# heracles-ec/heracles

Hardware: AMD Instinct MI355X
Metric: map->Cl pairs/sec + mixing-matrix build sec, nside=4096 lmax=6144 (higher is better)
Workload: dtype f64

## Files before the change

### heracles_amd/_lib.py

```python

from __future__ import annotations

import ctypes as C
import os
import threading

import numpy as np

_HERE = os.path.dirname(os.path.abspath(__file__))
_LIBNAME = os.environ.get("HX_LIBRARY") or os.path.join(_HERE, "libhxsht.so")
_lock = threading.Lock()
_lib = None

HX_OK = 0
HX_ERR_ARG, HX_ERR_NO_DEVICE, HX_ERR_HIP, HX_ERR_MEM, HX_ERR_UNSUPPORTED = -1, -2, -3, -4, -5

SYMBOLS = (
    "hx_version", "hx_last_error", "hx_device_count", "hx_init", "hx_set_stream",
    "hx_get_stream", "hx_set_async", "hx_synchronize", "hx_timer_start", "hx_timer_stop",
    "hx_profile_enable", "hx_profile_reset", "hx_profile_get", "hx_plan_create", "hx_set_max_lds_fft",
    "hx_plan_destroy", "hx_plan_scratch_bytes", "hx_plan_release_scratch", "hx_plan_set_leadin_resume", "hx_plan_set_leadin_cap", "hx_set_scratch_budget", "hx_plan_last_chunks", "hx_plan_mfma_flops", "hx_plan_executed_flops", "hx_executed_flops", "hx_measure_peaks", "hx_measured_mfma_clock", "hx_map2alm", "hx_map2alm_multi", "hx_map2alm_list", "hx_alm2map", "hx_copy",
    "hx_alm2cl_pairs", "hx_alm2cl_pairs_range", "hx_gauss_legendre", "hx_gauss_legendre_dd", "hx_wigner_d_table", "hx_mixmat",
    "hx_mixmat_eb", "hx_mixmat_eb_spin", "hx_mixmat_batch", "hx_mixctx_create", "hx_mixctx_apply", "hx_mixctx_apply_spin", "hx_mixctx_destroy", "hx_mixctx_set_bins", "hx_mixctx_apply_binned", "hx_mixctx_apply_binned_spin", "hx_cl2corr", "hx_corr2cl", "hx_cl2corr_cols", "hx_corr2cl_cols", "hx_cl2corr_cols_spin", "hx_corr2cl_cols_spin", "hx_xi_ratio", "hx_ang2pix_ring", "hx_map_values", "hx_ud_grade", "hx_reorder", "hx_matvec", "hx_pinv", "hx_alm_resample", "hx_region_maps", "hx_alm_subtract", "hx_fits_unpack_f64", "hx_fits_pack_f64", "hx_fits_unpack_columns",
    "hx_pointsht_create", "hx_pointsht_destroy", "hx_pointsht_info", "hx_pointsht_adjoint",
    "hx_pointsht_synthesis", "hx_pointsht_grids", "hx_pointgrid_gather", "hx_pointgrid_destroy",
    "hx_pixel_weights_size", "hx_pixel_weights_expand", "hx_pixel_weights_solve",
    "hx_ring_modes_size", "hx_ring_modes", "hx_legendre_from_modes", "hx_allgather_alms", "hx_host_alloc", "hx_host_free", "hx_mixmat_gemm_clock", "hx_mixmat_release", "hx_release_caches",
    "hx_cov_gram", "hx_cov_delete2", "hx_cov_shrink_sums",
    "hx_catmap_create", "hx_catmap_page", "hx_catmap_moments", "hx_catmap_finish", "hx_catmap_destroy",
    "hx_catalm_create", "hx_catalm_page", "hx_catalm_moments", "hx_catalm_finish", "hx_catalm_destroy",
    "hx_catmap_create_sel", "hx_catmap_page_sel", "hx_catmap_moments_sel", "hx_catmap_finish_sel", "hx_catmap_destroy_sel",
)


class HxError(RuntimeError):

# ... 24 lines not shown
        L = C.CDLL(_LIBNAME)
        vp, i, dp = C.c_void_p, C.c_int, C.c_void_p
        L.hx_version.restype = C.c_char_p
        L.hx_last_error.restype = C.c_char_p
        L.hx_get_stream.restype = vp
        L.hx_set_stream.argtypes = [vp]
        L.hx_plan_create.restype = vp
        L.hx_plan_create.argtypes = [i, i, i]
        L.hx_plan_destroy.argtypes = [vp]
        L.hx_plan_destroy.restype = None
        L.hx_plan_scratch_bytes.argtypes = [vp]
        L.hx_plan_scratch_bytes.restype = C.c_int64
        L.hx_plan_release_scratch.argtypes = [vp]
        L.hx_plan_set_leadin_resume.argtypes = [vp, i]
        L.hx_plan_set_leadin_cap.argtypes = [vp, C.c_int64]
        L.hx_set_scratch_budget.argtypes = [C.c_double]
        L.hx_plan_last_chunks.argtypes = [vp]
        L.hx_plan_mfma_flops.argtypes = [vp, i, i, C.POINTER(C.c_double)]
        L.hx_plan_executed_flops.argtypes = [vp, i, i, C.POINTER(C.c_double)]
        L.hx_executed_flops.argtypes = [C.POINTER(C.c_double), i]
        L.hx_measure_peaks.argtypes = [C.POINTER(C.c_double)]
        L.hx_measured_mfma_clock.restype = C.c_double
        L.hx_map2alm.argtypes = [vp, i, i, dp, dp, dp, dp, dp, i]
        L.hx_alm2map.argtypes = [vp, i, i, dp, dp]
        L.hx_map2alm_multi.argtypes = [vp, i, vp, vp, vp, vp, dp, dp, vp]
        L.hx_map2alm_list.argtypes = [vp, i, vp, vp, vp, dp, dp, dp, dp, i]
        L.hx_copy.argtypes = [vp, vp, C.c_int64]
        L.hx_alm2cl_pairs.argtypes = [i, vp, vp, i, i, vp, vp, dp]
        L.hx_alm2cl_pairs_range.argtypes = [i, vp, vp, i, i, vp, vp, i, i, i, dp]
        L.hx_gauss_legendre.argtypes = [i, dp, dp]
# ... 244 lines not shown
```

### heracles_amd/csrc/hx_analysis.hip

```cpp
#include <algorithm>
#include <cmath>
#include <cstdlib>
#include <cstring>

#include "hx_sht_common.h"

namespace hx {
using namespace hxfft;

constexpr int HALF_F = 1;
template <int SPIN>
struct LegCfg {
    static constexpr int NW = SPIN == 0 ? 16 : 8;
    static constexpr int NT = SPIN == 0 ? 1 : 2;
    static constexpr int NOP = SPIN == 0 ? 1 : 2;
    static constexpr int NPAR = (SPIN == 2 && HALF_F) ? 1 : 2;
};
int analysis_f_rows(int spin) { return spin == 0 ? LegCfg<0>::NPAR * LegCfg<0>::NOP : LegCfg<2>::NPAR * LegCfg<2>::NOP; }

struct LegParams {
    PlanDev P;
    const LegTask *__restrict__ tasks;
    const double *__restrict__ F;
    double *__restrict__ partial;
    int m0, ms;
    long long row0;
    int ng;
    int ncol;
    int pcol;
    const MTasks *__restrict__ of_m;
    const long long *__restrict__ arow;
    long long arow0;
    int add_all;
    const double *__restrict__ leadin;
    LegTask *tasks_out;
    double *leadin_out;
};

constexpr int COMB_NXCD = 8, COMB_XG = 4;
constexpr int COMB_TM = 16;
constexpr int COMB_IPT = 3;
constexpr int COMB_MPAD = 2;
static int combine_rp(int rowlen) { return rowlen <= 40 ? 8 : 4; }
static size_t combine_lds_bytes(int rp, int rowlen)
{
    return (size_t)COMB_TM * ((size_t)rp * rowlen + COMB_MPAD) * sizeof(double) + (size_t)COMB_TM * rp * sizeof(RingAtM) + COMB_TM * sizeof(int);
}
template <int SPIN, int RP>
__global__ __launch_bounds__(1024) void k_fourier_combine(PlanDev P, const double2 *__restrict__ Y, int ncomp, int ncol, int m0, int ms,
                                                         int nm, int kshift, int gx, int gy, const double *__restrict__ rw,
                                                         const LegTask *__restrict__ tasks, const MTasks *__restrict__ of_m,
// ... 121 lines not shown
template <int SPIN>
struct PipeCfg {
    static constexpr int NW = 4;
    static constexpr int RBS = SPIN == 0 ? 2 : 1;
    static constexpr int NCH = SPIN == 0 ? 2 : 1;
    static constexpr int NOP = SPIN == 0 ? 1 : 2;
};

__device__ __host__ inline int pipe_rho(int q, int k) { return 4 * q + k; }
__device__ __host__ inline int pipe_tile_idx(int c, int r) { return c * 32 + ((r ^ (c & 7)) * 2); }

constexpr int DUO_GAP = -1;
constexpr int DUO_PRIO = 1;
constexpr int DUO_ORDER = -1;
constexpr int DUO_SCALE_BITS2 = 100;
constexpr int DUO_SCALE_BITS0 = 300;

template <int K>
__device__ __forceinline__ double row_bcast(double v)
{
    double d;
    asm("v_mov_b64_dpp %0, %1 row_newbcast:%2 row_mask:0xf bank_mask:0xf" : "=v"(d) : "v"(v), "n"(K));
    return d;
}

template <int K>
__device__ __forceinline__ double row_bcast_fmac(double t, double p, double x)
{
    asm("v_fmac_f64_dpp %0, %1, %2 row_newbcast:%3 row_mask:0xf bank_mask:0xf" : "+v"(t) : "v"(p), "v"(x), "n"(K));
    return t;
}
// ... 84 lines not shown
    auto lds_barrier = []() __attribute__((always_inline)) {
        __builtin_amdgcn_s_waitcnt(0xc07f);
        __builtin_amdgcn_s_barrier();
    };
    int n_mf = 0, n_rec = 0;
    if (DUO_PRIO) __builtin_amdgcn_s_setprio(3);
    const int ti0 = SCOUT ? (int)blockIdx.y : 0, tis = SCOUT ? (int)gridDim.y : 1;
    for (int ti = ti0; ti < mt.count; ti += tis) {
        const LegTask task = SCOUT ? A.tasks_out[mt.first + ti] : A.tasks[mt.first + ti];
        first_group = ti == 0 && !A.add_all;
        const int bres = (RESUME && !SCOUT && A.leadin) ? task.pad : 0;
        int tid = threadIdx.x;
        asm volatile("; ring group" : "+v"(tid));
        const int w = tid >> 6, lane = tid & 63;
        const int ai = lane & 15, ak = lane >> 4;
        if (ti != ti0) __syncthreads();
        if (!SCOUT && bres > 0) {
            if (first_group) {
                double2 *z = reinterpret_cast<double2 *>(A.partial + orow * A.pcol);
                const long long nz = (long long)bres * LBLK * A.pcol / 2;
                for (long long i = tid; i < nz; i += 256) z[i] = make_double2(0.0, 0.0);
                asm volatile("s_waitcnt vmcnt(0)" ::: "memory");
            }
            if (bres >= nblk) continue;
        }

        const int rbi = SPIN == 0 ? 2 * w + (lane >> 5) : w;
        const int rpl = (task.rb0 + rbi) * RBLK + (lane & 31);
        const bool valid = rbi < task.nrb && rpl < P.nrp;
        const double x = valid ? P.z[rpl] : 0.0;
// ... 116 lines not shown
            return __all(dead) ? 1 : (__all(live) ? 3 : 2);
        };
        using I1 = std::integral_constant<int, 1>;
        using I2 = std::integral_constant<int, 2>;
        using I3 = std::integral_constant<int, 3>;

        const int fcol = tid & 15, fch = (tid >> 4) & 7, fpos = (tid >> 7) & 1;
        const int frow = (fch >> 1) + 8 * (fch & 1);
        const int qrow = tid / (4 * NXA), qcol = tid % (4 * NXA);
        double *pgrp = A.partial + (orow + (long long)bres * LBLK + 2 * frow + fpos) * A.pcol + fcol;
        double *pquad = A.partial + (orow + (long long)bres * LBLK + 2 * qrow) * A.pcol + NG * NCOL + qcol;
        double2 cnext[2] = {cfm[bres * LBLK], cfm[bres * LBLK + 16]};
        bool started = first_group;
        int nflush = 0;
        int woke = nblk;
        double svc[NCH], svp[NCH];
        int ssc[NCH];
        for (int b0 = bres; b0 < nblk; b0 += NSUB) {
            double4_t acc[NSUB][NG][2];
            double accx[NSUB][NXA][2];
            bool mine = false;
            if (SCOUT) {
#pragma unroll
                for (int c = 0; c < NCH; ++c) { svc[c] = vc[c]; svp[c] = vp[c]; ssc[c] = sc[c]; }
            }
#pragma unroll
            for (int sub = 0; sub < NSUB; ++sub) {
                const int b = b0 + sub;
#pragma unroll
                for (int g = 0; g < NG; ++g) acc[sub][g][0] = acc[sub][g][1] = (double4_t){0.0, 0.0, 0.0, 0.0};
#pragma unroll
                for (int g = 0; g < NXA; ++g) accx[sub][g][0] = accx[sub][g][1] = 0.0;
                if (b >= nblk) break;
                int rm = set_mode(b);
                const double2 cl[2] = {cnext[0], cnext[1]};
                if (rm == 3) recursion(I3{}, cl);
                else if (rm == 2) {
                    recursion(I2{}, cl);
                    if (SB != 300) {
                        bool lv = valid && sc[0] == 0;
                        if (NCH == 2) lv = lv || (valid && sc[NCH - 1] == 0);
                        if (!__any(lv)) rm = 1;
                    }
                } else recursion(I1{}, cl);
                cnext[0] = cfm[(b + 1) * LBLK];
                cnext[1] = cfm[(b + 1) * LBLK + 16];
                n_rec = __builtin_amdgcn_readfirstlane(n_rec + 1);
                mine = mine || rm >= 2;
                if (!SCOUT && rm >= 2) {
                    n_mf = __builtin_amdgcn_readfirstlane(n_mf + 1);
                    if (DUO_PRIO) __builtin_amdgcn_s_setprio(0);
                    constexpr int PF = 3;
                    auto a_fetch = [&](int sp) __attribute__((always_inline)) {
                        const int op = SPIN == 0 ? 0 : sp & 1, q = SPIN == 0 ? sp : sp >> 1;
                        const int c = SPIN == 0 ? (q >> 3) * 32 + pipe_rho(q & 7, ak) : op * 32 + pipe_rho(q, ak);
                        return *reinterpret_cast<const double2 *>(tw + pipe_tile_idx(c, ai));
                    };
                    double2 aq[PF + 1];
#pragma unroll
// ... 39 lines not shown
                                }
                            } else {
#pragma unroll
                                for (int g = 0; g < NG; ++g) acc[sub][g][pos] = __builtin_amdgcn_mfma_f64_16x16x4f64(a, fr[sp][HALFB ? 0 : pos][g], acc[sub][g][pos], 0, 0, 0);
#pragma unroll
                                for (int g = 0; g < NBX; ++g) accx[sub][g][pos] = __builtin_amdgcn_mfma_f64_4x4x4f64(a, frx[sp][HALFB ? 0 : pos][g], accx[sub][g][pos], 0, 0, 0);
                            }
                        }
                        __builtin_amdgcn_sched_barrier(0);
                    }
                    if (DUO_PRIO) __builtin_amdgcn_s_setprio(3);
                }
            }
            const bool two = NSUB > 1 && b0 + 1 < nblk;
            if (SCOUT) {
                if (lane == 0) lead_in[nflush & 1][w] = mine ? 1 : 0;
                lds_barrier();
                const int4 fl = *reinterpret_cast<const int4 *>(&lead_in[nflush & 1][0]);
                ++nflush;
                if (__builtin_amdgcn_readfirstlane(fl.x | fl.y | fl.z | fl.w) != 0) {
                    woke = b0;
                    break;
                }
                continue;
            }
            if (!started) {
                if (lane == 0) lead_in[nflush & 1][w] = mine ? 1 : 0;
                lds_barrier();
                const int4 fl = *reinterpret_cast<const int4 *>(&lead_in[nflush & 1][0]);
                ++nflush;
                started = __builtin_amdgcn_readfirstlane(fl.x | fl.y | fl.z | fl.w) != 0;
                if (!started) {
                    pgrp += (long long)NSUB * LBLK * A.pcol;
                    pquad += (long long)NSUB * LBLK * A.pcol;
                    continue;
                }
            }
#pragma unroll
// ... 25 lines not shown
                    put(pgrp + rsub + g * NCOL + 8 * (long long)A.pcol, (s4[0].y + s4[1].y) + (s4[2].y + s4[3].y));
                }
                if (NBX > 0 && tid < 64 * NBX) {
                    double2 s4[NW];
#pragma unroll
                    for (int ww = 0; ww < NW; ++ww) s4[ww] = *reinterpret_cast<const double2 *>(&tile[0][0] + ww * TW + sub * DSZ + DQ0 + tid * 2);
                    put(pquad + rsub, (s4[0].x + s4[1].x) + (s4[2].x + s4[3].x));
                    put(pquad + rsub + A.pcol, (s4[0].y + s4[1].y) + (s4[2].y + s4[3].y));
                }
            }
            pgrp += (long long)NSUB * LBLK * A.pcol;
            pquad += (long long)NSUB * LBLK * A.pcol;
            lds_barrier();
        }
        if (SCOUT) {
            if (woke > 0 && woke < nblk) {
                double *st = A.leadin_out + (long long)(mt.first + ti) * (NCH * 640) + tid;
#pragma unroll
                for (int c = 0; c < NCH; ++c) {
                    st[c * 640] = svc[c];
                    st[c * 640 + 256] = svp[c];
                    reinterpret_cast<int *>(st + c * 640 + 512 - tid)[tid] = ssc[c];
                }
            }
            if (tid == 0) A.tasks_out[mt.first + ti].pad = woke;
        }
    }
    if (!SCOUT && (threadIdx.x & 63) == 0) {
        atomicAdd(&g_exec_flops[0], (unsigned long long)n_mf * (32ull * (NG * 2048ull + NBX * 512ull)));
        atomicAdd(&g_exec_flops[1], (unsigned long long)n_rec * (64ull * LBLK * 4ull));
    }
// ... 135 lines not shown
        else return fail(HX_ERR_ARG, "legendre analysis: no two-group kernel for %d groups + %d blocks", sh.ng, sh.nbx);
        return HX_OK;
    }
    if (key == 10) hipLaunchKernelGGL((k_legendre_duo<SPIN, 1, 0, 2>), pgrid, db, 0, st, A, cn);
    else if (key == 11) hipLaunchKernelGGL((k_legendre_duo<SPIN, 1, 1, 2>), pgrid, db, 0, st, A, cn);
    else if (key == 20 && SPIN == 2) hipLaunchKernelGGL((k_legendre_duo<2, 2, 0, 2>), pgrid, db, 0, st, A, cn);
    else if (key == 12 && SPIN == 2) hipLaunchKernelGGL((k_legendre_duo<2, 1, 2, 2>), pgrid, db, 0, st, A, cn);
    else if (key == 21 && SPIN == 2) hipLaunchKernelGGL((k_legendre_duo<2, 2, 1, 2>), pgrid, db, 0, st, A, cn);
    else if (key == 20) hipLaunchKernelGGL((k_legendre_duo<SPIN, 2, 0>), pgrid, db, 0, st, A, cn);
    else if (key == 22 && SPIN == 2) hipLaunchKernelGGL((k_legendre_duo<2, 2, 2>), pgrid, db, 0, st, A, cn);
    else return fail(HX_ERR_ARG, "legendre analysis: no two-group kernel for %d groups + %d blocks", sh.ng, sh.nbx);
    return HX_OK;
}

constexpr long long LEADIN_CAP_BYTES = 8LL << 30;
static int leadin_table(hx_plan *pl, int spin, hx_plan::SpinData &sd, hx_plan::TaskSet &ts, const double **tab)
{
    *tab = nullptr;
    if (pl->leadin_resume < (spin == 0 ? 2 : 1) || ts.tasks.empty() || ts.leadin_skip) return HX_OK;
    if (ts.d_leadin.p) {
        *tab = ts.d_leadin.as<double>();
        return HX_OK;
    }
    const size_t per_task = (size_t)(spin == 0 ? PipeCfg<0>::NCH : PipeCfg<2>::NCH) * 640 * sizeof(double);
    const size_t bytes = ts.tasks.size() * per_task;
    size_t cap = (size_t)(pl->leadin_cap > 0 ? pl->leadin_cap : LEADIN_CAP_BYTES), fr = 0, tot = 0;
    if (hipMemGetInfo(&fr, &tot) == hipSuccess) cap = std::min(cap, fr / 10);
    else (void)hipGetLastError();
    if (bytes > cap) {
        ts.leadin_skip = true;
        return HX_OK;
    }
    if (ts.d_leadin.alloc(bytes) != HX_OK) {
        (void)hipGetLastError();
        ts.leadin_skip = true;
        return HX_OK;
    }
    LegParams A;
    A.P = pl->dev(); A.tasks = nullptr; A.F = nullptr; A.partial = nullptr;
    A.m0 = 0; A.ms = 1; A.row0 = 0; A.ng = 1; A.ncol = NCOL; A.pcol = NCOL;
    A.of_m = ts.d_of_m.as<MTasks>(); A.arow = ts.d_arow.as<long long>(); A.arow0 = 0; A.add_all = 1;
    A.leadin = nullptr; A.tasks_out = ts.d_tasks.as<LegTask>(); A.leadin_out = ts.d_leadin.as<double>();
    const dim3 grid((unsigned)(pl->lmax + 1), 8), db(256);
    if (spin == 0) hipLaunchKernelGGL((k_legendre_duo<0, 1, 0, 2, true>), grid, db, 0, rt().stream, A, sd.cn.as<double2>());
    else hipLaunchKernelGGL((k_legendre_duo<2, 1, 0, 2, true>), grid, db, 0, rt().stream, A, sd.cn.as<double2>());
    if (hipGetLastError() != hipSuccess) {
        ts.d_leadin.release();
        return fail(HX_ERR_HIP, "leadin_table: the scout launch failed");
    }
    *tab = ts.d_leadin.as<double>();
    return HX_OK;
}

static void launch_alm_reduce(hx_plan *pl, int spin, hx_plan::TaskSet &ts, long long row0, int m0, int ms, int nm, int nb, int ng, int pcol,
                              const double *d_fl, int add, double2 *d_alms, const double *al)
{
    const PlanDev P = pl->dev();
    const long long *arow = al ? ts.d_arow.as<long long>() : nullptr;
    if (spin == 0)
        hipLaunchKernelGGL(k_alm_reduce<0>, dim3(nm), dim3(256), 0, rt().stream, P, ts.d_tasks.as<LegTask>(), ts.d_of_m.as<MTasks>(), pl->partial.as<double>(),
                           row0, m0, ms, nb, ng, pcol, d_fl, add, d_alms, pl->nlm, arow, al);
    else
        hipLaunchKernelGGL(k_alm_reduce<2>, dim3(nm), dim3(256), 0, rt().stream, P, ts.d_tasks.as<LegTask>(), ts.d_of_m.as<MTasks>(), pl->partial.as<double>(),
                           row0, m0, ms, nb, ng, pcol, d_fl, add, d_alms, pl->nlm, arow, al);
}

template <int SPIN>
static int launch_chunk(hx_plan *pl, hx_plan::SpinData &sd, hx_plan::TaskSet &ts, int m0, int m1, int nb, const SweepShape &sh, const double *d_rw,
                        const double *d_fl, int add, double2 *d_alms, const double *leadin)
{
    const int ng = sh.ng + (sh.nbx > 0 ? 1 : 0), ncol = sh.ncol;
    const int pcol = sweep_pcol(sh);
    hipStream_t st = rt().stream;
    PlanDev P = pl->dev();
    const int t0 = ts.of_m[m0].first;
    const int t1 = ts.of_m[m1 - 1].first + ts.of_m[m1 - 1].count;
    const int ms = std::max(pl->m_step, 1), nm = (m1 - m0 + ms - 1) / ms;
    {
        ProfScope ps("fourier_combine");
        launch_fourier_combine<SPIN>(st, P, pl->Y.as<double2>(), nb, ncol, m0, ms, nm, d_rw, ts.d_tasks.as<LegTask>(), ts.d_of_m.as<MTasks>(),
                                     pl->F.as<double>(), 0, pl->nrp_pad / 32);
    }
    if (t1 > t0) {
        ProfScope ps("legendre_analysis");
        ProfScope ps2(SPIN == 0 ? "legendre_analysis_s0" : "legendre_analysis_s2");
        LegParams A;
        A.P = P; A.tasks = ts.d_tasks.as<LegTask>() + t0; A.F = pl->F.as<double>(); A.partial = pl->partial.as<double>();
        A.m0 = m0; A.ms = ms; A.row0 = ts.rows_before_m[m0]; A.ng = ng; A.ncol = ncol; A.pcol = pcol;
        A.of_m = ts.d_of_m.as<MTasks>(); A.arow = ts.d_arow.as<long long>(); A.arow0 = ts.arow[m0]; A.add_all = 0;
        A.tasks = ts.d_tasks.as<LegTask>();
        A.leadin = leadin; A.tasks_out = nullptr; A.leadin_out = nullptr;
        HX_TRY(launch_duo<SPIN>(sh, dim3((unsigned)nm), st, A, sd.cn.as<double2>()));
    }
    {
        ProfScope ps("alm_reduce");
        launch_alm_reduce(pl, SPIN, ts, ts.arow[m0], m0, ms, nm, nb, ng, pcol, d_fl, add, d_alms, sd.al.as<double>());
    }
    HX_HIP(hipGetLastError());
    return HX_OK;
}

static bool valu_batch(int spin, int nb) { return sweep_shape(spin, nb).valu != 0; }

static double analysis_budget(const hx_plan *pl)
{
    if (scratch_budget_bytes() > 0.0) return scratch_budget_bytes();
// ... 71 lines not shown
        return analysis_batch_valu(pl, spin, nb, d_maps, d_alms, d_rw, d_pw, d_fl, add, true);
    }
    if (valu_batch(spin, nb)) return analysis_batch_valu(pl, spin, nb, d_maps, d_alms, d_rw, d_pw, d_fl, add);
    const SweepShape sh = sweep_shape(spin, nb);
    hx_plan::TaskSet *ts = nullptr;
    hx_plan::SpinData *sd = nullptr;
    HX_TRY(spin_data(pl, spin, false, &sd));
    HX_TRY(task_set(pl, spin, false, one_set_task_blocks(spin), &ts));
    if (pl->hsrc == nullptr && pl->nssrc == nullptr) {
        HX_TRY(pl->Y.alloc(sizeof(double2) * (size_t)pl->ny * nb));
        HX_TRY(launch_ring_subdft_maps(pl, nb, d_maps, d_pw, pl->Y.as<double2>()));
    }
    std::vector<std::pair<int, int>> chunks;
    HX_TRY(plan_m_chunks(pl, (double)pl->nrp_pad * analysis_f_rows(spin) * sh.ncol * sizeof(double), ts->arow, sweep_pcol(sh) * sizeof(double), chunks));
    const double *leadin = nullptr;
    HX_TRY(leadin_table(pl, spin, *sd, *ts, &leadin));
    for (auto &ch : chunks) {
        if (spin == 0)
            HX_TRY(launch_chunk<0>(pl, *sd, *ts, ch.first, ch.second, nb, sh, d_rw, d_fl, add, d_alms, leadin));
        else
            HX_TRY(launch_chunk<2>(pl, *sd, *ts, ch.first, ch.second, nb, sh, d_rw, d_fl, add, d_alms, leadin));
    }
    return HX_OK;
}

bool analysis_can_stream(hx_plan *pl, int spin, int nb)
{
    if (!pl || pl->nside < 1 || pl->hsrc || pl->nssrc || pl->m_lo != 0 || pl->m_hi >= 0 || pl->m_step > 1) return false;
    if (nb < 1 || nb > analysis_max_comp(spin)) return false;
    const SweepShape sh = sweep_shape(spin, nb);
    if (!duo_shape(sh) || sh.valu) return false;
    const double f_bytes = (double)pl->nrp_pad * analysis_f_rows(spin) * sh.ncol * sizeof(double) * (pl->lmax + 1.0);
    const double p_bytes = 0.5 * (pl->lmax + 1.0) * (pl->lmax + 2.0 + LBLK) * sweep_pcol(sh) * sizeof(double);
    double budget = 80e9;
    if (scratch_budget_bytes() > 0.0) budget = scratch_budget_bytes();
    if (f_bytes + p_bytes > budget) return false;
// ... 4 lines not shown
    }
    const double y_bytes = (double)pl->ny * nb * sizeof(double2), stage_bytes = 2.0 * nb * (double)pl->npix * sizeof(double);
    const double held = (double)pl->F.bytes + (double)pl->partial.bytes + (double)pl->Y.bytes + (double)pl->stage[0].bytes + (double)pl->stage[1].bytes +
                        (double)pl->stage[2].bytes;
    return f_bytes + p_bytes + y_bytes + stage_bytes <= 0.95 * ((double)fr + held);
}

int analysis_stream_plan(hx_plan *pl, int spin, int nb, int nslab, StreamSweep &s)
{
    if (!analysis_can_stream(pl, spin, nb)) return fail(HX_ERR_ARG, "analysis_stream_plan: not a streamable sweep");
    HX_TRY(spin_data(pl, spin, false, &s.sd));
    HX_TRY(task_set(pl, spin, false, one_set_task_blocks(spin), &s.ts));
    hx_plan::TaskSet &ts = *s.ts;
    const SweepShape sh = sweep_shape(spin, nb);
    s.leadin = nullptr;
    s.pl = pl; s.spin = spin; s.nb = nb;
    const int nrb = (pl->nrp + RBLK - 1) / RBLK;
    std::vector<double> cum(nrb + 1, 0.0);
    for (int rb = 0; rb < nrb; ++rb) {
        double px = 0.0;
        for (int rp = rb * RBLK; rp < std::min((rb + 1) * RBLK, pl->nrp); ++rp) px += (rp == pl->nrp - 1 ? 4.0 : 8.0) * pl->h_nsub[rp];
        cum[rb + 1] = cum[rb] + px;
    }
    nslab = std::max(1, std::min(nslab, nrb));
    s.rp_edge.assign(1, 0);
    for (int k = 1; k < nslab; ++k) {
        const int rb = (int)(std::lower_bound(cum.begin(), cum.end(), cum[nrb] * k / nslab) - cum.begin());
        if (rb * RBLK > s.rp_edge.back() && rb < nrb) s.rp_edge.push_back(rb * RBLK);
    }
    s.rp_edge.push_back(nrb * RBLK);
// ... 7 lines not shown
            const int rb_hi = s.rp_edge[k + 1] / RBLK;
            MTasks &o = tab[(size_t)k * (lmax + 1) + m];
            o.first = t;
            while (t < mt.first + mt.count && ts.tasks[t].rb0 + ts.tasks[t].nrb <= rb_hi) ++t;
            o.count = t - o.first;
        }
        if (t != mt.first + mt.count) return fail(HX_ERR_ARG, "analysis_stream_plan: ring groups of m = %d left over", m);
    }
    HX_TRY(upload(s.d_of_m, tab));
    HX_TRY(pl->Y.alloc(sizeof(double2) * (size_t)pl->ny * nb));
    HX_TRY(pl->F.alloc((size_t)pl->nrp_pad * analysis_f_rows(spin) * sh.ncol * sizeof(double) * (size_t)(lmax + 1)));
    HX_TRY(pl->partial.alloc((size_t)ts.arow[lmax + 1] * sweep_pcol(sh) * sizeof(double)));
    return HX_OK;
}

int analysis_stream_leadin(StreamSweep &s) { return leadin_table(s.pl, s.spin, *s.sd, *s.ts, &s.leadin); }

int analysis_stream_start(StreamSweep &s)
{
    hx_plan *pl = s.pl;
    const SweepShape sh = sweep_shape(s.spin, s.nb);
    HX_HIP(hipMemsetAsync(pl->partial.p, 0, (size_t)s.ts->arow[pl->lmax + 1] * sweep_pcol(sh) * sizeof(double), rt().stream));
    pl->last_chunks = 1;
    return HX_OK;
}

template <int SPIN>
static int stream_slab(StreamSweep &s, int k)
{
    hx_plan *pl = s.pl;
    hx_plan::TaskSet &ts = *s.ts;
// ... 4 lines not shown
    PlanDev P = pl->dev();
    HX_TRY(launch_ring_subdft_maps(pl, s.nb, s.d_maps, s.d_pw, pl->Y.as<double2>(), rp_lo, std::min(rp_hi, pl->nrp)));
    {
        ProfScope ps("fourier_combine");
        const int tile_hi = k + 1 == s.nslab ? pl->nrp_pad / 32 : rp_hi / 32;
        launch_fourier_combine<SPIN>(st, P, pl->Y.as<double2>(), s.nb, sh.ncol, 0, 1, nm, s.d_rw, ts.d_tasks.as<LegTask>(), ts.d_of_m.as<MTasks>(),
                                     pl->F.as<double>(), rp_lo / 32, tile_hi - rp_lo / 32);
    }
    {
        ProfScope ps("legendre_analysis");
        ProfScope ps2(SPIN == 0 ? "legendre_analysis_s0" : "legendre_analysis_s2");
        LegParams A;
        A.P = P; A.tasks = ts.d_tasks.as<LegTask>(); A.F = pl->F.as<double>(); A.partial = pl->partial.as<double>();
        A.m0 = 0; A.ms = 1; A.row0 = 0; A.ng = ng; A.ncol = sh.ncol; A.pcol = sweep_pcol(sh);
        A.of_m = s.d_of_m.as<MTasks>() + (size_t)k * (lmax + 1); A.arow = ts.d_arow.as<long long>(); A.arow0 = 0; A.add_all = 1;
        A.leadin = s.leadin; A.tasks_out = nullptr; A.leadin_out = nullptr;
        HX_TRY(launch_duo<SPIN>(sh, dim3((unsigned)nm), st, A, s.sd->cn.as<double2>()));
    }
    HX_HIP(hipGetLastError());
    return HX_OK;
}

int analysis_stream_slab(StreamSweep &s, int k)
{
    if (k < 0 || k >= s.nslab) return fail(HX_ERR_ARG, "analysis_stream_slab: slab %d of %d", k, s.nslab);
    return s.spin == 0 ? stream_slab<0>(s, k) : stream_slab<2>(s, k);
}

int analysis_stream_end(StreamSweep &s)
{
    hx_plan *pl = s.pl;
// ... 52 lines not shown
}

extern "C" int hx_plan_executed_flops(hx_plan *pl, int spin, int ncomp, double *out2)
{
    using namespace hx;
    if (!out2) return fail(HX_ERR_ARG, "hx_plan_executed_flops: null output");
    HX_TRY(hx_plan_mfma_flops(pl, spin, ncomp, &out2[0]));
    double wave_blocks = 0.0;
    HX_TRY(flop_wave_blocks(pl, spin, &wave_blocks));
    const int nop = spin ? 2 : 1;
    int sweeps = 0;
    for (int c0 = 0, nb = 0; c0 < ncomp; c0 += nb, ++sweeps) nb = analysis_next_batch(spin, ncomp - c0);
    out2[1] = wave_blocks * sweeps * (double)RBLK * LBLK * nop * 4.0;
    return HX_OK;
}
```

### heracles_amd/csrc/hx_plan.hip

```cpp
#include <algorithm>
#include <cmath>

#include "hx_sht_common.h"

namespace hx {
__global__ void k_init_norm0(int lmax, double2 *__restrict__ coef, double *__restrict__ alpha)
{
    const int t = blockIdx.x * blockDim.x + threadIdx.x;
    const int m = t >> 1, par = t & 1;
    if (m > lmax) return;
    const double dm = m;
    auto a = [dm](double l) { return sqrt((4.0 * l * l - 1.0) / (l * l - dm * dm)); };
    double al = 1.0;
    for (int l = m + par; l <= lmax; l += 2) {
        const double dl = l;
        const double a1 = a(dl + 1.0), a2 = a(dl + 2.0);
        const double A = a1 * a2;
        double B = -a2 / a1;
        if (l > m) {
            const double a0 = a(dl);
            B -= a2 * a1 / (a0 * a0);
        }
        const double an = 0.25 * a2 * a1 / al;
        coef[almidx(lmax, l, m)] = make_double2(A * al / an, B * al / an);
// ... 199 lines not shown
{
    if (!pl) return fail(HX_ERR_ARG, "hx_plan_release_scratch: null plan");
    if (rt().ready) {
        HX_HIP(hipStreamSynchronize(rt().stream));
        if (rt().copy) HX_HIP(hipStreamSynchronize(rt().copy));
    }
    for (int i = 0; i < hx_plan::NSTAGE; ++i) pl->stage[i].release();
    pl->resid_maps.release();
    pl->Y.release();
    pl->F.release();
    pl->partial.release();
    pl->syn_tab.release();
    for (auto &sp : pl->spins)
        for (auto &kv : sp.second.tasks) {
            kv.second.d_leadin.release();
            kv.second.leadin_skip = false;
        }
    return HX_OK;
}

extern "C" int hx_plan_set_leadin_resume(hx_plan *pl, int on)
{
    if (!pl) return fail(HX_ERR_ARG, "hx_plan_set_leadin_resume: null plan");
    pl->leadin_resume = on < 0 ? 0 : (on > 2 ? 2 : on);
    return HX_OK;
}

extern "C" int hx_plan_set_leadin_cap(hx_plan *pl, int64_t bytes)
{
    if (!pl || bytes < 0) return fail(HX_ERR_ARG, "hx_plan_set_leadin_cap: null plan or negative cap");
    pl->leadin_cap = bytes;
    for (auto &sp : pl->spins)
        for (auto &kv : sp.second.tasks) kv.second.leadin_skip = false;
    return HX_OK;
}

extern "C" int64_t hx_plan_scratch_bytes(const hx_plan *pl)
{
    if (!pl) return 0;
    size_t spin_tables = 0;
    for (const auto &kv : pl->spins) {
        spin_tables += kv.second.cn.bytes + kv.second.al.bytes;
        for (const auto &ts : kv.second.tasks) spin_tables += ts.second.d_leadin.bytes;
    }
    return (int64_t)(pl->stage[0].bytes + pl->stage[1].bytes + pl->stage[2].bytes + pl->resid_maps.bytes + pl->Y.bytes + pl->F.bytes + pl->partial.bytes +
                     pl->bhat.bytes + pl->syn_tab.bytes + spin_tables);
}

extern "C" int hx_plan_last_chunks(const hx_plan *pl) { return pl ? pl->last_chunks : 0; }

namespace hx {
int spin_data(hx_plan *pl, int spin, bool generic, hx_plan::SpinData **out)
{
    const int lmax = pl->lmax, s = spin;
    if (generic ? (s < 1 || s > lmax) : (s != 0 && s != 2)) return fail(HX_ERR_ARG, "spin_data: spin %d at lmax %d", s, lmax);
    hx_plan::SpinData &sd = pl->spins[{s, generic}];
    *out = &sd;
    if (sd.cn.p && sd.al.p && (sd.kf.p || !generic)) return HX_OK;
// ... 109 lines not shown
```

### heracles_amd/csrc/hx_sht_common.h

```cpp
#pragma once
#include <map>
#include <vector>

#include "hx_common.h"
#include "hx_fft_core.h"

namespace hx {

typedef double double4_t __attribute__((ext_vector_type(4)));

constexpr int LBLK = 32;
constexpr int NCOL = 16;
constexpr int TABLE_PAD = 512;
constexpr int NGMAX = 2;
constexpr int RBLK = 32;
constexpr double SC_BIG = 0x1p+300, SC_SMALL = 0x1p-300;
constexpr int SPIN_ANY = -1;

struct LegTask {
    int m;
    int rb0;
    int nrb;
    int pad;
    long long pout;
// ... 284 lines not shown
    long long leadin_cap = 0;
    long long npix = 0, ny = 0, nlm = 0;
    size_t lds_fft = 0;
    hx::DevBuf z, omz, sth, rwdef, nsub, shifted, startN, startS, bhat_off, tw, bhat, mfac, kfac2;
    std::vector<double> h_sth, h_z;
    std::vector<int> h_nsub;
    std::vector<long long> h_startN, h_startS;
    struct TaskSet {
        std::vector<hx::LegTask> tasks;
        std::vector<hx::MTasks> of_m;
        std::vector<long long> rows_before_m;
        std::vector<long long> arow;
        hx::DevBuf d_tasks, d_of_m, d_arow;
        hx::DevBuf d_leadin;
        bool leadin_skip = false;
    };
    struct SpinData {
        hx::DevBuf cn, al, kf;
        hx::DevBuf syn_mlim;
        hx::DevBuf syn_boff;
        std::map<int, TaskSet> tasks;
    };
    std::map<std::pair<int, bool>, SpinData> spins;
    struct FftClass { int M, first, count, big; };
    std::vector<FftClass> fft_classes;
    hx::DevBuf fft_rp_list;
    hx::DevBuf fft_desc;
    std::vector<int> h_fft_rp_list;
    hx::DevBuf Y, F, partial, d_dbg, resid_maps, pw_sym;
    hx::DevBuf syn_tab;
// ... 25 lines not shown
bool analysis_generic_spin(int spin);
inline bool plan_generic_spin(const hx_plan *pl, int spin) { return (pl->hsrc || (pl->nside >= 1 && !pl->nssrc)) && analysis_generic_spin(spin); }
int analysis_max_comp(int spin);
int analysis_next_batch(int spin, int remaining);
int analysis_max_batch(int spin, int ncomp);
struct StreamSweep {
    hx_plan *pl = nullptr;
    int spin = 0, nb = 0, nslab = 0;
    const double *d_maps = nullptr, *d_rw = nullptr, *d_pw = nullptr, *d_fl = nullptr;
    double2 *d_alms = nullptr;
    std::vector<int> rp_edge;
    DevBuf d_of_m;
    hx_plan::SpinData *sd = nullptr;
    hx_plan::TaskSet *ts = nullptr;
    const double *leadin = nullptr;
};
bool analysis_can_stream(hx_plan *pl, int spin, int nb);
int analysis_stream_leadin(StreamSweep &s);
int analysis_stream_plan(hx_plan *pl, int spin, int nb, int nslab, StreamSweep &s);
int analysis_stream_start(StreamSweep &s);
int analysis_stream_slab(StreamSweep &s, int k);
int analysis_stream_end(StreamSweep &s);
int launch_valu_chunk(hx_plan *pl, int spin, const hx_plan::SpinData &sd, hx_plan::TaskSet &ts, int m0, int m1, int c0, const double *d_rw, bool generic = false);
int valu_task_blocks(int spin);
int valu_partial_cols(int spin);
int valu_operand_doubles(int spin);
int valu_exec_flops(unsigned long long *v, bool reset);
int synth_valu_max_units(int spin);
int synth_valu_task_blocks(int spin, int units);
int launch_synth_valu(hx_plan *pl, int spin, int units, const hx_plan::SpinData &sd, hx_plan::TaskSet &ts, const double2 *d_alm, double *d_Fv, bool generic = false);
// ... 7 lines not shown
```

### heracles_amd/sht.py

```python

from __future__ import annotations

import numpy as np

from . import _lib


def nlm(lmax: int) -> int:
    return (lmax + 1) * (lmax + 2) // 2


def _is_tensor(a) -> bool:
    return hasattr(a, "data_ptr") and not isinstance(a, np.ndarray)


class Plan:

    def __init__(self, nside: int, lmax: int, max_comp: int = 8):
        L = _lib.load()
        _lib.ensure_init()
        self.nside, self.lmax = int(nside), int(lmax)
        self.npix = 12 * self.nside**2
        self.nlm = nlm(self.lmax)
        self._h = L.hx_plan_create(self.nside, self.lmax, int(max_comp))
# ... 6 lines not shown
            self._h = None

    def release_scratch(self):
        _lib.check(_lib.load().hx_plan_release_scratch(self._h))

    def __del__(self):
        try:
            self.close()
        except Exception:
            pass

    def set_leadin_resume(self, on: bool = True, cap_bytes: int | None = None, spin0: bool = False):
        _lib.check(_lib.load().hx_plan_set_leadin_resume(self._h, (2 if spin0 else 1) if on else 0))
        if cap_bytes is not None:
            _lib.check(_lib.load().hx_plan_set_leadin_cap(self._h, int(cap_bytes)))

    @property
    def scratch_bytes(self) -> int:
        return int(_lib.load().hx_plan_scratch_bytes(self._h))

    @property
    def last_chunks(self) -> int:
        return int(_lib.load().hx_plan_last_chunks(self._h))

    def mfma_flops(self, spin, ncomp):
        import ctypes

        out = ctypes.c_double(0.0)
        _lib.check(_lib.load().hx_plan_mfma_flops(self._h, int(spin), int(ncomp), ctypes.byref(out)))
        return out.value
# ... 144 lines not shown
```

### include/hxsht.h

```cpp
#ifndef HXSHT_H
#define HXSHT_H
#include <stdint.h>
#ifdef __cplusplus
extern "C" {
#endif

#define HX_OK 0
#define HX_ERR_ARG (-1)
#define HX_ERR_NO_DEVICE (-2)
#define HX_ERR_HIP (-3)
#define HX_ERR_MEM (-4)
#define HX_ERR_UNSUPPORTED (-5)

typedef struct hx_plan hx_plan;

const char *hx_version(void);
const char *hx_last_error(void);
int hx_device_count(void);
int hx_init(int device);
int hx_set_stream(void *stream);
void *hx_get_stream(void);
int hx_set_async(int on);
int hx_synchronize(void);
int hx_copy(void *dst, const void *src, int64_t bytes);
// ... 1 lines not shown
int hx_host_free(void *p);

int hx_timer_start(void);
int hx_timer_stop(float *ms);
int hx_profile_enable(int on);
int hx_profile_reset(void);
int hx_profile_get(const char *name, int *launches, double *total_ms);

hx_plan *hx_plan_create(int nside, int lmax, int max_comp);
int hx_set_max_lds_fft(int points);
void hx_plan_destroy(hx_plan *plan);
int64_t hx_plan_scratch_bytes(const hx_plan *plan);
int hx_plan_release_scratch(hx_plan *plan);
int hx_plan_set_leadin_resume(hx_plan *plan, int on);
int hx_plan_set_leadin_cap(hx_plan *plan, int64_t bytes);
int hx_set_scratch_budget(double bytes);
int hx_plan_last_chunks(const hx_plan *plan);
int hx_measure_peaks(double *out4);
double hx_measured_mfma_clock(void);
double hx_mixmat_gemm_clock(void);
int hx_plan_mfma_flops(hx_plan *plan, int spin, int ncomp, double *flops);
int hx_plan_executed_flops(hx_plan *plan, int spin, int ncomp, double *out2);
int hx_executed_flops(double *out2, int reset);

int hx_map2alm(hx_plan *plan, int spin, int ncomp, const double *maps, double *alms,
               const double *ring_weights, const double *pix_weights, const double *fl,
               int niter);
int hx_alm2map(hx_plan *plan, int spin, int ncomp, const double *alms, double *maps);
int hx_map2alm_multi(hx_plan *plan, int njobs, const int *spins, const int *ncomps, const double *const *maps, double *const *alms,
                     const double *ring_weights, const double *pix_weights, const double *const *fls);
// ... 141 lines not shown
```

Measured before the change: 434.3.

## Precompute per-wave recursion mode boundaries in scout pass and reuse in sweeps

The scout Legendre kernel now records, for each ring group and wave, the first l-blocks where the recursion switches to the scaled (mode 2) and full (mode 3) variants, and stores them in a per-task-set device table. The main analysis sweeps read these boundaries instead of calling set_mode and doing a wave-wide vote on each block. This removes per-block mode decisions and the __any reduction from the hot loop. The scout now always runs, even with lead-in resume off, so it costs one extra launch and a small buffer. DUO_SCALE_BITS0 drops from 300 to 100, which changes the scaling threshold for spin 0, and a host API for inspecting the modes is added.

Result: no change. 436.2, median of 6 (+0.4%).

```diff
diff --git a/heracles_amd/_lib.py b/heracles_amd/_lib.py
--- a/heracles_amd/_lib.py
+++ b/heracles_amd/_lib.py
@@ -19,7 +19,7 @@
     "hx_version", "hx_last_error", "hx_device_count", "hx_init", "hx_set_stream",
     "hx_get_stream", "hx_set_async", "hx_synchronize", "hx_timer_start", "hx_timer_stop",
     "hx_profile_enable", "hx_profile_reset", "hx_profile_get", "hx_plan_create", "hx_set_max_lds_fft",
-    "hx_plan_destroy", "hx_plan_scratch_bytes", "hx_plan_release_scratch", "hx_plan_set_leadin_resume", "hx_plan_set_leadin_cap", "hx_set_scratch_budget", "hx_plan_last_chunks", "hx_plan_mfma_flops", "hx_plan_executed_flops", "hx_executed_flops", "hx_measure_peaks", "hx_measured_mfma_clock", "hx_map2alm", "hx_map2alm_multi", "hx_map2alm_list", "hx_alm2map", "hx_copy",
+    "hx_plan_destroy", "hx_plan_scratch_bytes", "hx_plan_release_scratch", "hx_plan_set_leadin_resume", "hx_plan_set_leadin_cap", "hx_plan_block_modes", "hx_set_scratch_budget", "hx_plan_last_chunks", "hx_plan_mfma_flops", "hx_plan_executed_flops", "hx_executed_flops", "hx_measure_peaks", "hx_measured_mfma_clock", "hx_map2alm", "hx_map2alm_multi", "hx_map2alm_list", "hx_alm2map", "hx_copy",
     "hx_alm2cl_pairs", "hx_alm2cl_pairs_range", "hx_gauss_legendre", "hx_gauss_legendre_dd", "hx_wigner_d_table", "hx_mixmat",
     "hx_mixmat_eb", "hx_mixmat_eb_spin", "hx_mixmat_batch", "hx_mixctx_create", "hx_mixctx_apply", "hx_mixctx_apply_spin", "hx_mixctx_destroy", "hx_mixctx_set_bins", "hx_mixctx_apply_binned", "hx_mixctx_apply_binned_spin", "hx_cl2corr", "hx_corr2cl", "hx_cl2corr_cols", "hx_corr2cl_cols", "hx_cl2corr_cols_spin", "hx_corr2cl_cols_spin", "hx_xi_ratio", "hx_ang2pix_ring", "hx_map_values", "hx_ud_grade", "hx_reorder", "hx_matvec", "hx_pinv", "hx_alm_resample", "hx_region_maps", "hx_alm_subtract", "hx_fits_unpack_f64", "hx_fits_pack_f64", "hx_fits_unpack_columns",
     "hx_pointsht_create", "hx_pointsht_destroy", "hx_pointsht_info", "hx_pointsht_adjoint",
@@ -74,6 +74,7 @@
         L.hx_plan_release_scratch.argtypes = [vp]
         L.hx_plan_set_leadin_resume.argtypes = [vp, i]
         L.hx_plan_set_leadin_cap.argtypes = [vp, C.c_int64]
+        L.hx_plan_block_modes.argtypes = [vp, i, C.POINTER(C.c_int32), C.c_int64, C.POINTER(C.c_int64)]
         L.hx_set_scratch_budget.argtypes = [C.c_double]
         L.hx_plan_last_chunks.argtypes = [vp]
         L.hx_plan_mfma_flops.argtypes = [vp, i, i, C.POINTER(C.c_double)]
diff --git a/heracles_amd/csrc/hx_analysis.hip b/heracles_amd/csrc/hx_analysis.hip
--- a/heracles_amd/csrc/hx_analysis.hip
+++ b/heracles_amd/csrc/hx_analysis.hip
@@ -33,8 +33,10 @@
     long long arow0;
     int add_all;
     const double *__restrict__ leadin;
+    const unsigned *__restrict__ modes;
     LegTask *tasks_out;
     double *leadin_out;
+    unsigned *modes_out;
 };
 
 constexpr int COMB_NXCD = 8, COMB_XG = 4;
@@ -186,7 +188,7 @@
 constexpr int DUO_PRIO = 1;
 constexpr int DUO_ORDER = -1;
 constexpr int DUO_SCALE_BITS2 = 100;
-constexpr int DUO_SCALE_BITS0 = 300;
+constexpr int DUO_SCALE_BITS0 = 100;
 
 template <int K>
 __device__ __forceinline__ double row_bcast(double v)
@@ -301,6 +303,12 @@
         asm volatile("; ring group" : "+v"(tid));
         const int w = tid >> 6, lane = tid & 63;
         const int ai = lane & 15, ak = lane >> 4;
+        int b2 = 0, b3 = 0;
+        if (!SCOUT) {
+            const unsigned mw = A.modes[(long long)(mt.first + ti) * NW + __builtin_amdgcn_readfirstlane(w)];
+            b2 = (int)(mw & 0xffffu);
+            b3 = (int)(mw >> 16);
+        }
         if (ti != ti0) __syncthreads();
         if (!SCOUT && bres > 0) {
             if (first_group) {
@@ -447,13 +455,14 @@
         bool started = first_group;
         int nflush = 0;
         int woke = nblk;
+        int wb2 = nblk, wb3 = nblk;
         double svc[NCH], svp[NCH];
         int ssc[NCH];
         for (int b0 = bres; b0 < nblk; b0 += NSUB) {
             double4_t acc[NSUB][NG][2];
             double accx[NSUB][NXA][2];
             bool mine = false;
-            if (SCOUT) {
+            if (SCOUT && woke == nblk) {
 #pragma unroll
                 for (int c = 0; c < NCH; ++c) { svc[c] = vc[c]; svp[c] = vp[c]; ssc[c] = sc[c]; }
             }
@@ -465,17 +474,21 @@
 #pragma unroll
                 for (int g = 0; g < NXA; ++g) accx[sub][g][0] = accx[sub][g][1] = 0.0;
                 if (b >= nblk) break;
-                int rm = set_mode(b);
+                int rm = SCOUT ? set_mode(b) : (b < b2 ? 1 : (b < b3 ? 2 : 3));
                 const double2 cl[2] = {cnext[0], cnext[1]};
                 if (rm == 3) recursion(I3{}, cl);
                 else if (rm == 2) {
                     recursion(I2{}, cl);
-                    if (SB != 300) {
+                    if (SCOUT) {
                         bool lv = valid && sc[0] == 0;
                         if (NCH == 2) lv = lv || (valid && sc[NCH - 1] == 0);
                         if (!__any(lv)) rm = 1;
                     }
                 } else recursion(I1{}, cl);
+                if (SCOUT) {
+                    if (rm >= 2 && wb2 > b) wb2 = b;
+                    if (rm == 3 && wb3 > b) wb3 = b;
+                }
                 cnext[0] = cfm[(b + 1) * LBLK];
                 cnext[1] = cfm[(b + 1) * LBLK + 16];
                 n_rec = __builtin_amdgcn_readfirstlane(n_rec + 1);
@@ -545,14 +558,14 @@
             }
             const bool two = NSUB > 1 && b0 + 1 < nblk;
             if (SCOUT) {
-                if (lane == 0) lead_in[nflush & 1][w] = mine ? 1 : 0;
-                lds_barrier();
-                const int4 fl = *reinterpret_cast<const int4 *>(&lead_in[nflush & 1][0]);
-                ++nflush;
-                if (__builtin_amdgcn_readfirstlane(fl.x | fl.y | fl.z | fl.w) != 0) {
-                    woke = b0;
-                    break;
+                if (woke == nblk) {
+                    if (lane == 0) lead_in[nflush & 1][w] = mine ? 1 : 0;
+                    lds_barrier();
+                    const int4 fl = *reinterpret_cast<const int4 *>(&lead_in[nflush & 1][0]);
+                    ++nflush;
+                    if (__builtin_amdgcn_readfirstlane(fl.x | fl.y | fl.z | fl.w) != 0) woke = b0;
                 }
+                if (woke < nblk && (wb3 < nblk || !__any(valid))) break;
                 continue;
             }
             if (!started) {
@@ -608,7 +621,8 @@
             lds_barrier();
         }
         if (SCOUT) {
-            if (woke > 0 && woke < nblk) {
+            if (lane == 0) A.modes_out[(long long)(mt.first + ti) * NW + w] = (unsigned)wb2 | ((unsigned)wb3 << 16);
+            if (A.leadin_out && woke > 0 && woke < nblk) {
                 double *st = A.leadin_out + (long long)(mt.first + ti) * (NCH * 640) + tid;
 #pragma unroll
                 for (int c = 0; c < NCH; ++c) {
@@ -774,41 +788,48 @@
 }
 
 constexpr long long LEADIN_CAP_BYTES = 8LL << 30;
-static int leadin_table(hx_plan *pl, int spin, hx_plan::SpinData &sd, hx_plan::TaskSet &ts, const double **tab)
+static int leadin_table(hx_plan *pl, int spin, hx_plan::SpinData &sd, hx_plan::TaskSet &ts, const double **tab, const unsigned **modes)
 {
     *tab = nullptr;
-    if (pl->leadin_resume < (spin == 0 ? 2 : 1) || ts.tasks.empty() || ts.leadin_skip) return HX_OK;
-    if (ts.d_leadin.p) {
-        *tab = ts.d_leadin.as<double>();
-        return HX_OK;
-    }
-    const size_t per_task = (size_t)(spin == 0 ? PipeCfg<0>::NCH : PipeCfg<2>::NCH) * 640 * sizeof(double);
-    const size_t bytes = ts.tasks.size() * per_task;
-    size_t cap = (size_t)(pl->leadin_cap > 0 ? pl->leadin_cap : LEADIN_CAP_BYTES), fr = 0, tot = 0;
-    if (hipMemGetInfo(&fr, &tot) == hipSuccess) cap = std::min(cap, fr / 10);
-    else (void)hipGetLastError();
-    if (bytes > cap) {
-        ts.leadin_skip = true;
-        return HX_OK;
-    }
-    if (ts.d_leadin.alloc(bytes) != HX_OK) {
-        (void)hipGetLastError();
-        ts.leadin_skip = true;
-        return HX_OK;
-    }
-    LegParams A;
-    A.P = pl->dev(); A.tasks = nullptr; A.F = nullptr; A.partial = nullptr;
-    A.m0 = 0; A.ms = 1; A.row0 = 0; A.ng = 1; A.ncol = NCOL; A.pcol = NCOL;
-    A.of_m = ts.d_of_m.as<MTasks>(); A.arow = ts.d_arow.as<long long>(); A.arow0 = 0; A.add_all = 1;
-    A.leadin = nullptr; A.tasks_out = ts.d_tasks.as<LegTask>(); A.leadin_out = ts.d_leadin.as<double>();
-    const dim3 grid((unsigned)(pl->lmax + 1), 8), db(256);
-    if (spin == 0) hipLaunchKernelGGL((k_legendre_duo<0, 1, 0, 2, true>), grid, db, 0, rt().stream, A, sd.cn.as<double2>());
-    else hipLaunchKernelGGL((k_legendre_duo<2, 1, 0, 2, true>), grid, db, 0, rt().stream, A, sd.cn.as<double2>());
-    if (hipGetLastError() != hipSuccess) {
-        ts.d_leadin.release();
-        return fail(HX_ERR_HIP, "leadin_table: the scout launch failed");
-    }
-    *tab = ts.d_leadin.as<double>();
+    *modes = nullptr;
+    if (ts.tasks.empty()) return HX_OK;
+    if ((pl->lmax >> 5) + 1 > 0xffff) return fail(HX_ERR_ARG, "mode_table: %d blocks of 32 l do not fit 16 bits", (pl->lmax >> 5) + 1);
+    bool new_states = false;
+    if (pl->leadin_resume >= (spin == 0 ? 2 : 1) && !ts.leadin_skip && !ts.d_leadin.p) {
+        const size_t per_task = (size_t)(spin == 0 ? PipeCfg<0>::NCH : PipeCfg<2>::NCH) * 640 * sizeof(double);
+        const size_t bytes = ts.tasks.size() * per_task;
+        size_t cap = (size_t)(pl->leadin_cap > 0 ? pl->leadin_cap : LEADIN_CAP_BYTES), fr = 0, tot = 0;
+        if (hipMemGetInfo(&fr, &tot) == hipSuccess) cap = std::min(cap, fr / 10);
+        else (void)hipGetLastError();
+        if (bytes > cap) ts.leadin_skip = true;
+        else if (ts.d_leadin.alloc(bytes) != HX_OK) {
+            (void)hipGetLastError();
+            ts.leadin_skip = true;
+        } else new_states = true;
+    }
+    const bool new_modes = !ts.d_modes.p;
+    if (new_modes && ts.d_modes.alloc(ts.tasks.size() * PipeCfg<0>::NW * sizeof(unsigned)) != HX_OK) {
+        if (new_states) ts.d_leadin.release();
+        return fail(HX_ERR_HIP, "mode_table: no room for the block modes of %zu ring groups", ts.tasks.size());
+    }
+    if (new_states || new_modes) {
+        LegParams A;
+        A.P = pl->dev(); A.tasks = nullptr; A.F = nullptr; A.partial = nullptr;
+        A.m0 = 0; A.ms = 1; A.row0 = 0; A.ng = 1; A.ncol = NCOL; A.pcol = NCOL;
+        A.of_m = ts.d_of_m.as<MTasks>(); A.arow = ts.d_arow.as<long long>(); A.arow0 = 0; A.add_all = 1;
+        A.leadin = nullptr; A.modes = nullptr; A.tasks_out = ts.d_tasks.as<LegTask>();
+        A.leadin_out = new_states ? ts.d_leadin.as<double>() : nullptr; A.modes_out = ts.d_modes.as<unsigned>();
+        const dim3 grid((unsigned)(pl->lmax + 1), 8), db(256);
+        if (spin == 0) hipLaunchKernelGGL((k_legendre_duo<0, 1, 0, 2, true>), grid, db, 0, rt().stream, A, sd.cn.as<double2>());
+        else hipLaunchKernelGGL((k_legendre_duo<2, 1, 0, 2, true>), grid, db, 0, rt().stream, A, sd.cn.as<double2>());
+        if (hipGetLastError() != hipSuccess) {
+            if (new_states) ts.d_leadin.release();
+            if (new_modes) ts.d_modes.release();
+            return fail(HX_ERR_HIP, "leadin_table: the scout launch failed");
+        }
+    }
+    *modes = ts.d_modes.as<unsigned>();
+    if (pl->leadin_resume >= (spin == 0 ? 2 : 1) && !ts.leadin_skip && ts.d_leadin.p) *tab = ts.d_leadin.as<double>();
     return HX_OK;
 }
 
@@ -827,7 +848,7 @@
 
 template <int SPIN>
 static int launch_chunk(hx_plan *pl, hx_plan::SpinData &sd, hx_plan::TaskSet &ts, int m0, int m1, int nb, const SweepShape &sh, const double *d_rw,
-                        const double *d_fl, int add, double2 *d_alms, const double *leadin)
+                        const double *d_fl, int add, double2 *d_alms, const double *leadin, const unsigned *modes)
 {
     const int ng = sh.ng + (sh.nbx > 0 ? 1 : 0), ncol = sh.ncol;
     const int pcol = sweep_pcol(sh);
@@ -849,7 +870,7 @@
         A.m0 = m0; A.ms = ms; A.row0 = ts.rows_before_m[m0]; A.ng = ng; A.ncol = ncol; A.pcol = pcol;
         A.of_m = ts.d_of_m.as<MTasks>(); A.arow = ts.d_arow.as<long long>(); A.arow0 = ts.arow[m0]; A.add_all = 0;
         A.tasks = ts.d_tasks.as<LegTask>();
-        A.leadin = leadin; A.tasks_out = nullptr; A.leadin_out = nullptr;
+        A.leadin = leadin; A.modes = modes; A.tasks_out = nullptr; A.leadin_out = nullptr; A.modes_out = nullptr;
         HX_TRY(launch_duo<SPIN>(sh, dim3((unsigned)nm), st, A, sd.cn.as<double2>()));
     }
     {
@@ -951,12 +972,13 @@
     std::vector<std::pair<int, int>> chunks;
     HX_TRY(plan_m_chunks(pl, (double)pl->nrp_pad * analysis_f_rows(spin) * sh.ncol * sizeof(double), ts->arow, sweep_pcol(sh) * sizeof(double), chunks));
     const double *leadin = nullptr;
-    HX_TRY(leadin_table(pl, spin, *sd, *ts, &leadin));
+    const unsigned *modes = nullptr;
+    HX_TRY(leadin_table(pl, spin, *sd, *ts, &leadin, &modes));
     for (auto &ch : chunks) {
         if (spin == 0)
-            HX_TRY(launch_chunk<0>(pl, *sd, *ts, ch.first, ch.second, nb, sh, d_rw, d_fl, add, d_alms, leadin));
+            HX_TRY(launch_chunk<0>(pl, *sd, *ts, ch.first, ch.second, nb, sh, d_rw, d_fl, add, d_alms, leadin, modes));
         else
-            HX_TRY(launch_chunk<2>(pl, *sd, *ts, ch.first, ch.second, nb, sh, d_rw, d_fl, add, d_alms, leadin));
+            HX_TRY(launch_chunk<2>(pl, *sd, *ts, ch.first, ch.second, nb, sh, d_rw, d_fl, add, d_alms, leadin, modes));
     }
     return HX_OK;
 }
@@ -991,6 +1013,7 @@
     hx_plan::TaskSet &ts = *s.ts;
     const SweepShape sh = sweep_shape(spin, nb);
     s.leadin = nullptr;
+    s.modes = nullptr;
     s.pl = pl; s.spin = spin; s.nb = nb;
     const int nrb = (pl->nrp + RBLK - 1) / RBLK;
     std::vector<double> cum(nrb + 1, 0.0);
@@ -1028,7 +1051,7 @@
     return HX_OK;
 }
 
-int analysis_stream_leadin(StreamSweep &s) { return leadin_table(s.pl, s.spin, *s.sd, *s.ts, &s.leadin); }
+int analysis_stream_leadin(StreamSweep &s) { return leadin_table(s.pl, s.spin, *s.sd, *s.ts, &s.leadin, &s.modes); }
 
 int analysis_stream_start(StreamSweep &s)
 {
@@ -1063,7 +1086,8 @@
         A.P = P; A.tasks = ts.d_tasks.as<LegTask>(); A.F = pl->F.as<double>(); A.partial = pl->partial.as<double>();
         A.m0 = 0; A.ms = 1; A.row0 = 0; A.ng = ng; A.ncol = sh.ncol; A.pcol = sweep_pcol(sh);
         A.of_m = s.d_of_m.as<MTasks>() + (size_t)k * (lmax + 1); A.arow = ts.d_arow.as<long long>(); A.arow0 = 0; A.add_all = 1;
-        A.leadin = s.leadin; A.tasks_out = nullptr; A.leadin_out = nullptr;
+        if (!s.modes && !s.ts->tasks.empty()) return fail(HX_ERR_ARG, "analysis_stream_slab: analysis_stream_leadin has not run");
+        A.leadin = s.leadin; A.modes = s.modes; A.tasks_out = nullptr; A.leadin_out = nullptr; A.modes_out = nullptr;
         HX_TRY(launch_duo<SPIN>(sh, dim3((unsigned)nm), st, A, s.sd->cn.as<double2>()));
     }
     HX_HIP(hipGetLastError());
@@ -1146,3 +1170,32 @@
     out2[1] = wave_blocks * sweeps * (double)RBLK * LBLK * nop * 4.0;
     return HX_OK;
 }
+
+extern "C" int hx_plan_block_modes(hx_plan *pl, int spin, int32_t *out, int64_t cap, int64_t *ntasks)
+{
+    using namespace hx;
+    if (!pl || !ntasks || (spin != 0 && spin != 2) || pl->nside < 1) return fail(HX_ERR_ARG, "hx_plan_block_modes: bad arguments");
+    HX_TRY(ensure_ready());
+    hx_plan::TaskSet *ts = nullptr;
+    hx_plan::SpinData *sd = nullptr;
+    HX_TRY(spin_data(pl, spin, false, &sd));
+    HX_TRY(task_set(pl, spin, false, one_set_task_blocks(spin), &ts));
+    const size_t n = ts->tasks.size();
+    *ntasks = (int64_t)n;
+    if (!out || n == 0) return HX_OK;
+    if (cap < (int64_t)n) return fail(HX_ERR_ARG, "hx_plan_block_modes: room for %lld of %zu ring groups", (long long)cap, n);
+    const double *tab = nullptr;
+    const unsigned *modes = nullptr;
+    HX_TRY(leadin_table(pl, spin, *sd, *ts, &tab, &modes));
+    std::vector<LegTask> tk(n);
+    std::vector<unsigned> md(n * PipeCfg<0>::NW);
+    HX_HIP(hipMemcpyAsync(tk.data(), ts->d_tasks.p, n * sizeof(LegTask), hipMemcpyDeviceToHost, rt().stream));
+    HX_HIP(hipMemcpyAsync(md.data(), modes, md.size() * sizeof(unsigned), hipMemcpyDeviceToHost, rt().stream));
+    HX_HIP(hipStreamSynchronize(rt().stream));
+    for (size_t t = 0; t < n; ++t) {
+        int32_t *o = out + 8 * t;
+        o[0] = tk[t].m; o[1] = tk[t].rb0; o[2] = tk[t].nrb; o[3] = tk[t].pad;
+        for (int w = 0; w < PipeCfg<0>::NW; ++w) o[4 + w] = (int32_t)md[t * PipeCfg<0>::NW + w];
+    }
+    return HX_OK;
+}
diff --git a/heracles_amd/csrc/hx_plan.hip b/heracles_amd/csrc/hx_plan.hip
--- a/heracles_amd/csrc/hx_plan.hip
+++ b/heracles_amd/csrc/hx_plan.hip
@@ -237,6 +237,7 @@
     for (auto &sp : pl->spins)
         for (auto &kv : sp.second.tasks) {
             kv.second.d_leadin.release();
+            kv.second.d_modes.release();
             kv.second.leadin_skip = false;
         }
     return HX_OK;
@@ -264,7 +265,7 @@
     size_t spin_tables = 0;
     for (const auto &kv : pl->spins) {
         spin_tables += kv.second.cn.bytes + kv.second.al.bytes;
-        for (const auto &ts : kv.second.tasks) spin_tables += ts.second.d_leadin.bytes;
+        for (const auto &ts : kv.second.tasks) spin_tables += ts.second.d_leadin.bytes + ts.second.d_modes.bytes;
     }
     return (int64_t)(pl->stage[0].bytes + pl->stage[1].bytes + pl->stage[2].bytes + pl->resid_maps.bytes + pl->Y.bytes + pl->F.bytes + pl->partial.bytes +
                      pl->bhat.bytes + pl->syn_tab.bytes + spin_tables);
diff --git a/heracles_amd/csrc/hx_sht_common.h b/heracles_amd/csrc/hx_sht_common.h
--- a/heracles_amd/csrc/hx_sht_common.h
+++ b/heracles_amd/csrc/hx_sht_common.h
@@ -322,6 +322,7 @@
         hx::DevBuf d_tasks, d_of_m, d_arow;
         hx::DevBuf d_leadin;
         bool leadin_skip = false;
+        hx::DevBuf d_modes;
     };
     struct SpinData {
         hx::DevBuf cn, al, kf;
@@ -377,6 +378,7 @@
     hx_plan::SpinData *sd = nullptr;
     hx_plan::TaskSet *ts = nullptr;
     const double *leadin = nullptr;
+    const unsigned *modes = nullptr;
 };
 bool analysis_can_stream(hx_plan *pl, int spin, int nb);
 int analysis_stream_leadin(StreamSweep &s);
diff --git a/heracles_amd/sht.py b/heracles_amd/sht.py
--- a/heracles_amd/sht.py
+++ b/heracles_amd/sht.py
@@ -44,6 +44,26 @@
         _lib.check(_lib.load().hx_plan_set_leadin_resume(self._h, (2 if spin0 else 1) if on else 0))
         if cap_bytes is not None:
             _lib.check(_lib.load().hx_plan_set_leadin_cap(self._h, int(cap_bytes)))
+
+    def block_modes(self, spin):
+        import ctypes as C
+
+        import numpy as np
+
+        n = C.c_int64()
+        _lib.check(_lib.load().hx_plan_block_modes(self._h, int(spin), None, 0, C.byref(n)))
+        raw = np.zeros((n.value, 8), dtype=np.int32)
+        if n.value:
+            _lib.check(_lib.load().hx_plan_block_modes(self._h, int(spin), raw.ctypes.data_as(C.POINTER(C.c_int32)), n.value, C.byref(n)))
+        return self.unpack_block_modes(raw)
+
+    @staticmethod
+    def unpack_block_modes(raw):
+        import numpy as np
+
+        raw = np.asarray(raw)
+        words = raw[:, 4:8].astype(np.int64) & 0xFFFFFFFF
+        return np.concatenate([raw[:, :4].astype(np.int64), words & 0xFFFF, words >> 16], axis=1)
 
     @property
     def scratch_bytes(self) -> int:
diff --git a/include/hxsht.h b/include/hxsht.h
--- a/include/hxsht.h
+++ b/include/hxsht.h
@@ -39,6 +39,7 @@
 int hx_plan_release_scratch(hx_plan *plan);
 int hx_plan_set_leadin_resume(hx_plan *plan, int on);
 int hx_plan_set_leadin_cap(hx_plan *plan, int64_t bytes);
+int hx_plan_block_modes(hx_plan *plan, int spin, int32_t *out, int64_t cap, int64_t *ntasks);
 int hx_set_scratch_budget(double bytes);
 int hx_plan_last_chunks(const hx_plan *plan);
 int hx_measure_peaks(double *out4);
```
